# rflamino/monte_carlo_retirement

Hardware: AMD Instinct MI355X
Metric: paths/sec (whole node), config.json scenario, 833-month paths, success-count only (higher is better)
Workload: dtype f64

## Files before the change

monte_carlo_retirement_amd/csrc/build.py:

```python

from __future__ import annotations

import os
import shutil
import subprocess
import sys

HERE = os.path.dirname(os.path.abspath(__file__))
SOURCES = ["mcr_hip.hip", "mcr_aggregate.hip"]
HEADERS = ["mcr_device.h", "mcr_math.h", "mcr_tables.h", "mcr_numpy_rng.h", "mcr_numpy_tables.h", "mcr_screen.h", "mcr_host.h", os.path.join("..", "..", "include", "mcr.h")]
TARGET = os.path.join(HERE, "libmcr_hip.so")
ARCH = "gfx950"
FLAGS = ["-O3", "-std=c++17", "-fPIC", "-shared", "-ffp-contract=off", f"--offload-arch={ARCH}",
         "-Wall", "-Wno-unused-function"]


def hipcc() -> str:
    for cand in (os.environ.get("HIPCC"), shutil.which("hipcc"), "/opt/rocm/bin/hipcc"):
        if cand and os.path.exists(cand):
            return cand
    raise RuntimeError("hipcc not found (need ROCm)")


def is_stale() -> bool:
    if not os.path.exists(TARGET):
        return True
    t = os.path.getmtime(TARGET)
    deps = [os.path.join(HERE, s) for s in SOURCES + HEADERS] + [os.path.abspath(__file__)]
    return any(os.path.getmtime(d) > t for d in deps)


PER_SOURCE_FLAGS = {"mcr_hip.hip": ["-Xarch_device", "-fno-honor-nans"]}


def build(force: bool = False, verbose: bool = False, extra_flags=(), variant: str = "") -> str:
    if variant:
        return _build_to(os.path.join(HERE, f"libmcr_hip_{variant}.so"), f"_{variant}", verbose, extra_flags)
    if not force and not is_stale():
        return TARGET
    return _build_to(TARGET, "", verbose, extra_flags)


def _build_to(target: str, obj_suffix: str, verbose: bool, extra_flags) -> str:
    compile_flags = [f for f in FLAGS if f != "-shared"]
    objs = []
    for src in SOURCES:
        obj = os.path.join(HERE, src.replace(".hip", f"{obj_suffix}.o"))
        cmd = [hipcc(), *compile_flags, *PER_SOURCE_FLAGS.get(src, []), *extra_flags, "-c", "-o", obj, os.path.join(HERE, src)]
        if verbose:
            print(" ".join(cmd), flush=True)
        subprocess.check_call(cmd)
        objs.append(obj)
    cmd = [hipcc(), "-shared", "-fPIC", f"--offload-arch={ARCH}", "-o", target, *objs]
    if verbose:
        print(" ".join(cmd), flush=True)
    subprocess.check_call(cmd)
    return target


if __name__ == "__main__":
    build(force="--force" in sys.argv, verbose=True,
          extra_flags=["-Rpass-analysis=kernel-resource-usage"] if "--verbose" in sys.argv else [])
    print(TARGET)
```

monte_carlo_retirement_amd/csrc/mcr_device.h:

```cpp
#pragma once

#include <hip/hip_runtime.h>
#include <stdint.h>

#include "../../include/mcr.h"
#include "mcr_math.h"

#define MCR_MASKED_MOVE do { if (MM) asm volatile(""); } while (0)
namespace mcr {

constexpr double kEps = MCR_SMALL_EPSILON;
constexpr int kMPY = MCR_MONTHS_PER_YEAR;
constexpr int kBlock = 256;

struct DevStream {
    double amount;
    double keep;
    double amount_keep;
    int32_t start_month;
    int32_t end_month;
    int32_t indexed;
    int32_t lock_slot;
};
typedef const __attribute__((address_space(4))) DevStream* DevStreamTable;
// ... 532 lines not shown
        if (dust_s) { MCR_MASKED_MOVE; nbs = 0.0; ncs = 0.0; }
        if (dust_b) { MCR_MASKED_MOVE; nbb = 0.0; ncb = 0.0; }
        if (act) {
            MCR_MASKED_MOVE;
            if (sell1) { MCR_MASKED_MOVE; b1 = nbs; c1 = ncs; b2 = nbb; c2 = ncb; }
            else { MCR_MASKED_MOVE; b1 = nbb; c1 = ncb; b2 = nbs; c2 = ncs; }
        }
    }
}

template <bool TAXED, bool MM = true>
__device__ __forceinline__ void rebalance_path(const LaneParams& P, double& b1, double& c1, double& b2, double& c2) {
    const double total = b1 + b2;
    const double drift1 = b1 - total * P.alloc1;
    if ((total > kEps) && (fabs(drift1) > kEps)) {
        MCR_MASKED_MOVE;
        const bool sell1 = drift1 > 0.0;
        const double drift2 = b2 - total * P.alloc2;
        const double bs = sell1 ? b1 : b2, cs = sell1 ? c1 : c2;
        const double drift = sell1 ? drift1 : drift2;
        const double alloc_s = sell1 ? P.alloc1 : P.alloc2;
        const double rate_s = sell1 ? P.real_rate1 : P.real_rate2;
        const double inv_bs = recip_nr<false>(bs);
        double gross_sale;
        if (TAXED) {
            const double gain_fraction = div_by(fmax(0.0, bs - cs), bs, inv_bs);
            const double tax_per_dollar = gain_fraction * rate_s;
            const double denom = fmax(kEps, 1.0 - alloc_s * tax_per_dollar);
            gross_sale = fmin(bs, fdiv<false>(drift, denom));
        } else {
            gross_sale = fmin(bs, drift);
        }
        const double fraction_sold = div_by(gross_sale, bs, inv_bs);
        const double basis_removed = cs * fraction_sold;
        double net_purchase = gross_sale;
        if (TAXED) {
            const double taxable_gain = fmax(0.0, gross_sale - basis_removed);
            net_purchase = gross_sale - taxable_gain * rate_s;
        }
        const double nbs = bs - gross_sale;
        const double ncs = cs - basis_removed;
        double r1b = b1 + net_purchase, r1c = c1 + net_purchase;
        double r2b = b2 + net_purchase, r2c = c2 + net_purchase;
        if (sell1) { MCR_MASKED_MOVE; r1b = nbs; r1c = ncs; }
        else { MCR_MASKED_MOVE; r2b = nbs; r2c = ncs; }
        if (r1b <= kEps) { MCR_MASKED_MOVE; r1b = 0.0; r1c = 0.0; }
        if (r2b <= kEps) { MCR_MASKED_MOVE; r2b = 0.0; r2c = 0.0; }
        b1 = r1b; c1 = r1c; b2 = r2b; c2 = r2c;
    }
}

enum { kMonthEqualRates = 1 };

enum { kStreamsInRegs = 1 };


__device__ __forceinline__ bool wave_any(bool c) { return __builtin_amdgcn_ballot_w64(c) != 0ull; }

template <bool T1, bool T2 = T1, bool MM = true, bool UNIFORM = false>
__device__ __forceinline__ double capacity_tol(double b1, double c1, double r1, double b2, double c2, double r2) {
    double v1 = b1, v2 = b2;
    if (T1) v1 = __builtin_fma(-fmax(0.0, b1 - c1), r1, b1);
    if (T2) v2 = __builtin_fma(-fmax(0.0, b2 - c2), r2, b2);
    if (!UNIFORM) {
        if (b1 <= kEps) { MCR_MASKED_MOVE; v1 = 0.0; }
        if (b2 <= kEps) { MCR_MASKED_MOVE; v2 = 0.0; }
    }
    return v1 + v2;
}
template <bool MM = true, bool UNIFORM = false>
__device__ __forceinline__ void sell_fraction_tol(double phi, double& b1, double& c1, double& b2, double& c2) {
    double nb1 = __builtin_fma(-b1, phi, b1), nc1 = __builtin_fma(-c1, phi, c1);
    double nb2 = __builtin_fma(-b2, phi, b2), nc2 = __builtin_fma(-c2, phi, c2);
    if (!UNIFORM || wave_any(fmin(nb1, nb2) <= kEps)) {
        if (nb1 <= kEps) { MCR_MASKED_MOVE; nb1 = 0.0; nc1 = 0.0; }
        if (nb2 <= kEps) { MCR_MASKED_MOVE; nb2 = 0.0; nc2 = 0.0; }
    }
    if (!UNIFORM) {
        if (b1 <= kEps) { MCR_MASKED_MOVE; nb1 = b1; nc1 = c1; }
        if (b2 <= kEps) { MCR_MASKED_MOVE; nb2 = b2; nc2 = c2; }
    }
    b1 = nb1; c1 = nc1; b2 = nb2; c2 = nc2;
}
template <bool TAXED, bool MM = true, bool UNIFORM = false, bool EQR = false>
__device__ __forceinline__ void rebalance_tol(const DevParams& P, const LaneParams& L, double& b1, double& c1, double& b2, double& c2) {
    const double total = b1 + b2;
    const double drift1 = __builtin_fma(-total, P.alloc1, b1);
    if (UNIFORM && wave_any(fmin(total, fabs(drift1)) <= kEps)) {
        rebalance_tol<TAXED, MM, false, EQR>(P, L, b1, c1, b2, c2);
        return;
    }
    if (UNIFORM || ((total > kEps) && (fabs(drift1) > kEps))) {
        MCR_MASKED_MOVE;
        const bool sell1 = drift1 > 0.0;
        const double bs = sell1 ? b1 : b2, cs = sell1 ? c1 : c2;
        const double drift = fabs(drift1);
        double fraction_sold, net_purchase;
        if (TAXED) {
            const double rate_s = EQR ? L.real_rate1 : sell1 ? L.real_rate1 : L.real_rate2;
            const double ar_s = sell1 ? L.alloc1 : L.alloc2;
            const double G = fmax(0.0, bs - cs);
            fraction_sold = fmin(1.0, drift * recip_nr<false>(__builtin_fma(-ar_s, G, bs)));
            net_purchase = fraction_sold * __builtin_fma(-G, rate_s, bs);
        } else {
            fraction_sold = fmin(1.0, drift * recip_nr<false>(bs));
            net_purchase = fraction_sold * bs;
        }
        const double nbs = __builtin_fma(-bs, fraction_sold, bs);
        const double ncs = __builtin_fma(-cs, fraction_sold, cs);
        double r1b = b1 + net_purchase, r1c = c1 + net_purchase;
        double r2b = b2 + net_purchase, r2c = c2 + net_purchase;
        if (sell1) { MCR_MASKED_MOVE; r1b = nbs; r1c = ncs; }
        else { MCR_MASKED_MOVE; r2b = nbs; r2c = ncs; }
        if (!UNIFORM || wave_any(fmin(r1b, r2b) <= kEps)) {
            if (r1b <= kEps) { MCR_MASKED_MOVE; r1b = 0.0; r1c = 0.0; }
            if (r2b <= kEps) { MCR_MASKED_MOVE; r2b = 0.0; r2c = 0.0; }
        }
        b1 = r1b; c1 = r1c; b2 = r2b; c2 = r2c;
    }
}

template <bool STRICT = true, bool TAXED = true, bool ANNUAL = true, bool T1 = TAXED, bool T2 = TAXED, bool MM = true, bool TOL = false, bool EQR = false>
__device__ __forceinline__ bool annual_gain_taxes(const DevParams& P, const LaneParams& L, double& b1, double& c1,
                                                  double& b2, double& c2, double gain1, double gain2) {
    bool tax_failed = false;
    if (ANNUAL && P.any_annual_tax) {
        const double due1 = fmax(0.0, gain1) * P.annual_rate1;
        const double due2 = fmax(0.0, gain2) * P.annual_rate2;
        const double total_due = due1 + due2;
        const double cap1 = net_liquidation_value<STRICT, T1, MM>(b1, c1, L.real_rate1);
        const double cap2 = net_liquidation_value<STRICT, T2, MM>(b2, c2, L.real_rate2);
        const double cap = cap1 + cap2;
        const double pay = fmin(total_due, cap);
        tax_failed = pay < total_due - kEps;
        if (cap > kEps && pay > 0.0) {
            const double share1 = fdiv<STRICT>(cap1, cap);
            const double share2 = 1.0 - share1;
            double g, net1, net2;
            withdraw<STRICT, T1, MM>(b1, c1, pay * share1, L.real_rate1, g, net1);
            withdraw<STRICT, T2, MM>(b2, c2, pay * share2, L.real_rate2, g, net2);
            tax_failed = tax_failed || (net1 + net2 < total_due - kEps);
        }
    }
    if (STRICT) rebalance<true, TAXED, MM>(L, b1, c1, b2, c2);
    else if (TOL) rebalance_tol<TAXED, MM, false, EQR>(P, L, b1, c1, b2, c2);
    else rebalance_path<TAXED, MM>(L, b1, c1, b2, c2);
    return tax_failed;
}

template <bool ANNUAL = true, bool TOL = false>
__device__ __forceinline__ void market_step(double g1, double ginf, double g2, double& b1, double& b2,
                                            double& gacc1, double& gacc2, double& infl) {
    if (ANNUAL) {
        if (TOL) {
            gacc1 = __builtin_fma(b1, g1 - 1.0, gacc1);
            gacc2 = __builtin_fma(b2, g2 - 1.0, gacc2);
        } else {
            gacc1 += b1 * (g1 - 1.0);
            gacc2 += b2 * (g2 - 1.0);
        }
    }
    b1 *= g1;
    b2 *= g2;
    infl *= ginf;
}

}
```

monte_carlo_retirement_amd/csrc/mcr_hip.hip:

```cpp

#include <hip/hip_runtime.h>

#include <climits>
#include <cmath>
#include <cstdarg>
#include <cstdio>
#include <cstdlib>
#include <cstring>
#include <algorithm>
#include <mutex>
#include <thread>
#include <type_traits>
#include <utility>
#include <vector>

#include "mcr_device.h"
#include "mcr_numpy_rng.h"
#include "mcr_screen.h"
#include "mcr_host.h"

namespace mcr {

constexpr int kMaxSegments = 8;
constexpr int kRngHistorySchemes = 3;
struct KernelIO {
    uint64_t seed;
    uint64_t path_begin;
    uint64_t n_paths;
    const double* injected;
    mcr_outputs out;
    uint32_t stream_id;
    union { uint32_t n_entropy; uint32_t history_months; };
    union { uint32_t entropy[MCR_MAX_ENTROPY_WORDS]; struct { uint32_t history_block, history_scheme; }; };
    uint64_t child_offset;
    union {
        const uint32_t* path_seeds;
        const double* history;
    };
    double* snap;
    int64_t snap_stride;
    int32_t n_snap;
    int32_t snap_months[MCR_MAX_PROBE_CANDIDATES];
    int32_t cand_out[MCR_MAX_PROBE_CANDIDATES];
    int32_t seg_n_split, seg_n_full, seg_q;
    int32_t seg_blocks_per_cand;
    double* seg_state;
    int32_t seg_year[kMaxSegments + 1];
    int32_t seg_bid_base;
    unsigned int* seg_flags;
    int32_t seg_max_polls;
    int32_t fan_n;
    struct YearBins {
        const double* edges;
        const double* wr_edges;
        unsigned long long* trajectory;
        unsigned long long* real_trajectory;
        unsigned long long* wr;
        unsigned long long* final_success;
        int32_t n_bins, n_wr_bins;
    };
    struct FanRows {
        int64_t fan_stream_word;
        double* final_balance;
        double* years_to_ruin;
        int64_t row_stride;
    };
    struct RuleIO {
        double upper, lower, keep, grow, floor, ceiling;
        unsigned long long* year_counts;
        double* multipliers;
        int64_t stride;
    };
    struct FanRuleRows {
        FanRows rows;
        unsigned long long* year_counts;
    };
    union {
        double fan_expenses[MCR_MAX_EXPENSE_FANOUT];
        YearBins yb;
        int32_t fan_stream;
        FanRows fan_rows;
        struct { const uint32_t* path_list; const uint32_t* path_list_count; };
        RuleIO rule;
        FanRuleRows fan_rule;
    };
    uint64_t* fan_masks;
};
static_assert(sizeof(KernelIO::YearBins) <= sizeof(double) * MCR_MAX_EXPENSE_FANOUT, "the yearly-bins block must fit the bytes it overlays");
static_assert(sizeof(KernelIO::FanRows) <= sizeof(double) * MCR_MAX_EXPENSE_FANOUT, "the outcome rows must fit the bytes they overlay");
static_assert(sizeof(KernelIO::RuleIO) <= sizeof(double) * MCR_MAX_EXPENSE_FANOUT, "the spending rule must fit the bytes it overlays");
static_assert(sizeof(KernelIO::FanRuleRows) <= sizeof(double) * MCR_MAX_EXPENSE_FANOUT && offsetof(KernelIO::FanRuleRows, rows) == 0,
              "the rule fan-out's rows must fit the bytes they overlay, the outcome rows where every outcome probe reads them");
constexpr size_t kKernelIOArgOffset = (sizeof(DevParams) + alignof(KernelIO) - 1) / alignof(KernelIO) * alignof(KernelIO);
template <typename T> __device__ __forceinline__ T late_arg(size_t offset_in_io) {
    typedef const char __attribute__((address_space(4)))* KernArg;
    return *(const T __attribute__((address_space(4)))*)((KernArg)__builtin_amdgcn_kernarg_segment_ptr() + kKernelIOArgOffset + offset_in_io);
}
struct GridCell {
    DevParams p;
// ... 209 lines not shown
__device__ __forceinline__ void rule_year_binned(RuleState& r, const YearBinsRuleState& B, int year, bool valid, bool alive, double b1, double b2, double infl, uint64_t li) {
    rule_year_from(r, B.R, year, valid, alive, b1, b2, infl, li);
    if (B.L.mbins && valid && alive)
        atomicAdd(&B.L.buf[(B.k & 1) * B.L.row + 2 * B.L.cells + B.L.wcells + year_bins_cell(B.L.medges, B.L.mn, r.m)], 1u);
}
__device__ __forceinline__ void rule_bins_begin(YearBinsRuleState& B, const void* record) {
    const RuleBinsRecord* const rec = static_cast<const RuleBinsRecord*>(record);
    B.R.upper = rec->upper; B.R.lower = rec->lower; B.R.keep = rec->keep; B.R.grow = rec->grow; B.R.floor = rec->floor; B.R.ceiling = rec->ceiling;
    B.R.year_counts = rec->year_counts;
}
__device__ __forceinline__ void rule_bins_begin(YearBinsState&, const void*) {}
template <typename IO>
__device__ __forceinline__ void rule_year(NoRuleState&, const IO&, int, bool, bool, double, double, double, uint64_t) {}
template <typename IO>
__device__ __forceinline__ void rule_pad(const RuleState&, const IO& io, int year, bool valid, uint64_t li) {
    if (io.rule.multipliers && valid) store_bits(&io.rule.multipliers[(int64_t)year * io.rule.stride + (int64_t)li], kNanBits);
}
template <typename IO>
__device__ __forceinline__ void rule_pad(const NoRuleState&, const IO&, int, bool, uint64_t) {}
__device__ __forceinline__ void income_put(DevStream& S, const IncomeRegs& R) {
    S.amount = R.amount; S.amount_keep = R.amount_keep; S.start_month = R.start_month; S.end_month = R.end_month;
}

template <int MODE, int RNG, int TAXED, bool ANNUAL, bool INJ = false, int PHASE = 0, bool SPLIT = false, bool XS = false, bool EXACT = kExactMonthDefault, int GF = 0, int MF = 0, int SF = 0, bool OUT = false, bool LIST = false, int NPROD = 1, bool RULE = false>
__global__ __launch_bounds__((PHASE == 5 || PHASE == 6 || PHASE == 7 || PHASE == 8 || PHASE == 9 || PHASE == 10 || PHASE == 11) ? 64 * (MCR_MAX_EXPENSE_FANOUT + 1) : NPROD == 2 ? 3 * 64 : SPLIT ? 2 * kBlock : kBlock, SPLIT ? 4 : (MODE == 0 && RNG == 0 && (PHASE == 0 || PHASE == 3 || PHASE == 4)) ? 6 : ((MODE == 1 || MODE == 2) && RNG == 0 && !INJ) ? 5 : 4) void path_kernel(const DevParams P_arg, const KernelIO io,
                                                         const DevParams* __restrict__ cand_params) {
    static_assert(MODE != 3 || (PHASE == 0 && !SPLIT && !INJ), "the yearly-bins form is a whole-path launch on the engine's own streams");
    static_assert(!SPLIT || (MODE == 0 && RNG == 0 && !INJ), "the producer / consumer split exists for the count-only Philox variants");
    static_assert(!XS || (PHASE == 0 && !SPLIT && TAXED == 3 && ANNUAL), "extended stream lists run the generic whole-path form");
    static_assert(PHASE != 5 || SPLIT, "the expense fan-out is a producer / consumer form");
    static_assert(PHASE != 6 || SPLIT, "the grid fan-out is a producer / consumer form");
    static_assert(PHASE != 7 || SPLIT, "the contribution fan-out is a producer / consumer form");
    static_assert(PHASE != 8 || SPLIT, "the scenario fan-out is a producer / consumer form");
    static_assert(PHASE != 9 || SPLIT, "the assumption fan-out is a producer / consumer form");
    static_assert(PHASE != 10 || SPLIT, "the income fan-out is a producer / consumer form");
    static_assert(PHASE != 11 || (SPLIT && RULE), "the rule fan-out is a producer / consumer form of the rule kernels");
    static_assert(!OUT || PHASE == 8 || PHASE == 9 || PHASE == 10 || PHASE == 11, "outcome rows exist for the scenario, assumption, income and rule fan-outs");
    static_assert(!LIST || (MODE == 0 && RNG == (int)MCR_RNG_PHILOX && !ANNUAL && !INJ && PHASE == 0 && !XS), "path lists exist for the whole-path count-only Philox launches, split or not");
    static_assert(NPROD == 1 || (NPROD == 2 && SPLIT && LIST), "two producers exist for the split re-run of a screened launch");
    static_assert(!RULE || (RNG == (int)MCR_RNG_PHILOX && TAXED == 3 && !INJ && !XS && EXACT == kExactMonthDefault && GF == 0 && MF == 0 && SF == 0 && !LIST && NPROD == 1 &&
                            (((MODE == 0 || MODE == 1 || MODE == 3) && PHASE == 0 && !SPLIT && !OUT) || (MODE == 0 && PHASE == 11 && SPLIT) || (MODE == 0 && PHASE == 6 && SPLIT && !OUT))),
                  "the spending rule exists for the plain whole-path Philox launches, count-only, summary and yearly bins, and for the rule and the rule grid fan-outs, on the generic tax mask");
    constexpr bool kExpFan = PHASE == 5 || PHASE == 6;
    constexpr bool kConFan = PHASE == 7;
    constexpr bool kAsmFan = PHASE == 9;
    constexpr bool kStreamRegs = SPLIT && !kAsmFan && !(LIST && (SF & kStreamsInRegs) != 0);
    constexpr bool kIncFan = PHASE == 10;
    constexpr bool kRuleFan = PHASE == 11;
    constexpr bool kScnFan = PHASE == 8 || kAsmFan || kIncFan || kRuleFan;
    constexpr bool kFan = kExpFan || kConFan || kScnFan;
    constexpr bool kGrid = PHASE == 6;
    constexpr bool kRuleGrid = kGrid && RULE;
    constexpr bool kWaveRule = kRuleFan || kRuleGrid;
    constexpr bool kCand = PHASE == 2 || PHASE == 4 || kExpFan;
    constexpr bool kSliced = PHASE == 3 || PHASE == 4;
    constexpr bool kSIR = (SF & kStreamsInRegs) != 0;
    constexpr bool kScalarCounters = MODE == 0 && RNG == 0 && !ANNUAL && !INJ && (PHASE == 0 || PHASE == 3) && !SPLIT && !XS &&
                                     (kSIR || !(GF == (kGrowthNarrowExp | kGrowthRhoZero) && MF == 0));
    [[maybe_unused]] std::conditional_t<kScalarCounters, MonthCounters, NoMonthCounters> SC;
    [[maybe_unused]] std::conditional_t<kSIR, StreamRegs, NoStreamRegs> SR;
    [[maybe_unused]] std::conditional_t<kIncFan, IncomeRegs, NoIncomeRegs> IR;
    [[maybe_unused]] std::conditional_t<OUT, RuinMonth, NoRuinMonth> RM;
    [[maybe_unused]] std::conditional_t<RULE, RuleState, NoRuleState> RS;
    [[maybe_unused]] std::conditional_t<kWaveRule, FanRule, NoFanRule> FR;
    static_assert(!kSliced || (RNG == 0 && !INJ && !SPLIT && !XS), "time-sliced blocks exist for the plain Philox variants");
    static_assert(PHASE != 4 || MODE == 0, "the search probes count only");
    static_assert(TAXED >= 0 && TAXED <= 3, "TAXED is a two-bit mask");
    constexpr bool T1 = (TAXED & 1) != 0, T2 = (TAXED & 2) != 0, TANY = TAXED != 0;
    static_assert(!EXACT || XS || kExactMonthDefault, "the exact month is instantiated for the generic variants only");
    static_assert(GF == 0 || GF == kGrowthNarrowExp || GF == (kGrowthNarrowExp | kGrowthRhoZero), "growth forms: masks 0, 1 and 3");
    static_assert(GF == 0 || (MODE == 0 && RNG == (int)MCR_RNG_PHILOX && !ANNUAL && !INJ && (PHASE == 0 || PHASE == 3) && !SPLIT && !XS),
                  "growth forms exist for the per-path Philox count-only launches (kPerPathPhilox), whole path or time-sliced");
    static_assert(MF == 0 || MF == kMonthEqualRates, "month forms: masks 0 and 1");
    static_assert(MF == 0 || (MODE == 0 && RNG == (int)MCR_RNG_PHILOX && !ANNUAL && !INJ && (PHASE == 0 || PHASE == 3) && (!SPLIT || LIST) && !XS && !EXACT),
                  "month forms exist for the kernels that have growth forms and for the split re-run of a screened launch, in the tolerance form of the month");
    static_assert(!(MF & kMonthEqualRates) || TAXED == 3, "equal realized-gains rates: both assets are taxed");
    constexpr bool EQR = (MF & kMonthEqualRates) != 0;
    static_assert(SF == 0 || SF == kStreamsInRegs, "stream forms: masks 0 and 1");
    static_assert(SF == 0 || (MODE == 0 && RNG == (int)MCR_RNG_PHILOX && !ANNUAL && !INJ && (PHASE == 0 || PHASE == 3) && (!SPLIT || LIST) && !XS && !EXACT),
                  "stream forms exist for the kernels that have growth forms and for the split re-run of a screened launch, in the tolerance form of the month");
    constexpr bool TOL = !EXACT;
    constexpr bool MM = !SPLIT || kFan || NPROD == 2 || LIST;
    constexpr bool kFastMonth = TOL && MM && kUniformFixups;
    constexpr int kPaths = (kFan || NPROD == 2) ? 64 : kBlock;
    const int kThreads = kFan ? (int)blockDim.x : NPROD == 2 ? 3 * 64 : SPLIT ? 2 * kBlock : kBlock;
    const int tid = SPLIT ? (int)(threadIdx.x & (kPaths - 1)) : (int)threadIdx.x;
    const int fan_j = kFan ? __builtin_amdgcn_readfirstlane((int)(threadIdx.x >> 6)) : 0;
    const bool producer = kFan ? fan_j == io.fan_n : (SPLIT && threadIdx.x >= (unsigned)kPaths);
    int seg = -1, seg_block = 0;
    unsigned int path_block = blockIdx.x, cand = (PHASE == 2 || kGrid) ? blockIdx.y : 0u;
    if (kSliced) {
        const int S = io.seg_n_split, F = io.seg_n_full, bid = (int)blockIdx.x + io.seg_bid_base;
        unsigned int lb = (unsigned)bid;
        if (bid < S) { seg = 0; seg_block = bid; }
        else if (bid >= S + F) { const int k = bid - S - F; seg = 1 + k / S; seg_block = k % S; lb = (unsigned)seg_block; }
        if (PHASE == 4) { cand = lb / (unsigned)io.seg_blocks_per_cand; path_block = lb % (unsigned)io.seg_blocks_per_cand; }
        else path_block = lb;
    }
    if constexpr (LIST) {
        if ((uint64_t)blockIdx.x * kPaths >= (uint64_t)*io.path_list_count) return;
    }
    const GridCell* cell = kRuleGrid ? &(reinterpret_cast<const RuleGridCell*>(cand_params) + cand)->cell
                           : kGrid ? reinterpret_cast<const GridCell*>(cand_params) + cand : nullptr;
    const DevParams& P = kGrid ? cell->p : (kCand && !kFan) ? cand_params[cand] : P_arg;
    const int snap_c = kGrid ? cell->snap : (int)cand;
    constexpr bool kStaged = RNG == (int)MCR_RNG_PHILOX && !INJ;
    constexpr bool kHistory = (RNG == (int)MCR_RNG_HISTORY || RNG == kRngHistorySchemes) && !INJ;
    __shared__ __align__(16) double tab_s[kHistory ? 1 : kTabDoubles];
    constexpr int kStageLen = (kAsmFan ? kPartsPerPair : 6) * kPaths;
    constexpr int kStageRing = SPLIT ? 2 : 1;
    __shared__ __align__(16) double stage_s[kStaged ? kStageRing * kStageLen : 1];
    constexpr bool kBins = MODE == 3;
    constexpr bool kSumLds = (MODE == 1 || MODE == 2) && kStaged;
    __shared__ __align__(16) double sum_s[kSumLds ? 3 * kBlock : 1];
    extern __shared__ __align__(16) unsigned char smem_raw[];
#ifdef MCR_K1_TIMELINE
    const unsigned long long tl_t0 = wall_clock64();
#endif
    double* tab = kHistory ? reinterpret_cast<double*>(smem_raw) : tab_s;
    load_math_tables<(GF & kGrowthNarrowExp) != 0>(tab, threadIdx.x, kThreads);
    ZigTables zig{nullptr, nullptr, nullptr, nullptr};
    if (RNG == (int)MCR_RNG_NUMPY) { zig = load_zig_tables(smem_raw, threadIdx.x, kThreads); zig.math_tab = tab; }
    [[maybe_unused]] const double* const hist_tab = reinterpret_cast<const double*>(smem_raw);
    [[maybe_unused]] std::conditional_t<kHistory, HistoryCursor, NoHistoryCursor> HC;
    if constexpr (kHistory) {
        constexpr int kRowsPerThread = MCR_MAX_HISTORY_MONTHS / kBlock;
        static_assert(kRowsPerThread * kBlock == MCR_MAX_HISTORY_MONTHS, "every row of the longest record has a thread");
        HC = history_cursor();
        __syncthreads();
        const int H = (int)io.history_months;
        double g[kRowsPerThread][3];
#pragma unroll
        for (int i = 0; i < kRowsPerThread; ++i) {
            const int k = (int)threadIdx.x + i * kBlock;
            g[i][0] = g[i][1] = g[i][2] = 0.0;
            if (k < H) {
                const double ze = io.history[3 * k + 0], zi = io.history[3 * k + 1], zp = io.history[3 * k + 2];
                g[i][0] = monthly_gross(P.a1, P.b1, ze, tab);
                g[i][1] = monthly_gross(P.ainf, P.binf, zi, tab);
                g[i][2] = g[i][1] * monthly_gross(P.aprem, P.bprem, zp, tab);
            }
        }
        __syncthreads();
        double* const G = reinterpret_cast<double*>(smem_raw);
#pragma unroll
        for (int i = 0; i < kRowsPerThread; ++i) {
            const int k = (int)threadIdx.x + i * kBlock;
            if (k < H) { G[3 * k + 0] = g[i][0]; G[3 * k + 1] = g[i][1]; G[3 * k + 2] = g[i][2]; }
        }
    }
    double* stage = stage_s + (kStaged ? tid : 0);
    double* sum_col = sum_s + (kSumLds ? tid : 0);
    double* lock_lds = reinterpret_cast<double*>(smem_raw + (RNG == (int)MCR_RNG_NUMPY ? (size_t)kZigLdsBytes
                                                             : kHistory ? (size_t)io.history_months * 3u * sizeof(double) : (size_t)0));
    unsigned int* blk = reinterpret_cast<unsigned int*>(lock_lds + (size_t)P.n_lock_slots * kPaths * (kFan ? io.fan_n : 1));
    if (kFan && !producer) lock_lds += (size_t)fan_j * P.n_lock_slots * kPaths;
    const int ry = P.retirement_years;
    const int n_blk = kFan ? MCR_MAX_EXPENSE_FANOUT : 1 + (ry + 2) + (ry + 1);
    const int n_hist = ((PHASE == 0 || PHASE == 3) && io.out.hist_bins != nullptr) ? io.out.hist_n_bins : 0;
    for (int k = threadIdx.x; k < n_blk + n_hist; k += kThreads) blk[k] = 0u;
    constexpr bool kBinsRule = kBins && RULE;
    [[maybe_unused]] std::conditional_t<kBins, std::conditional_t<kBinsRule, YearBinsRuleState, YearBinsState>, NoYearBins> YB;
    if constexpr (kBins) {
        year_bins_plan(YB.L, io.yb, cand_params, blk + n_blk + n_hist);
        rule_bins_begin(YB, cand_params);
        YB.k = 0; YB.last = 0.0;
// ... 200 lines not shown
        c1 = b1; c2 = b2;
        contrib = rec->monthly_contribution;
        scn_expenses = rec->monthly_expenses;
    } else if constexpr (kRuleFan) {
        const RuleRecord* const rec = reinterpret_cast<const RuleRecord*>(cand_params) + fan_j;
        const double rec_balance = rec->initial_balance;
        b1 = rec_balance * P.alloc1;
        b2 = rec_balance - b1;
        c1 = b1; c2 = b2;
        contrib = rec->monthly_contribution;
        scn_expenses = rec->monthly_expenses;
        FR.upper = rec->upper; FR.lower = rec->lower; FR.keep = rec->keep; FR.grow = rec->grow; FR.floor = rec->floor; FR.ceiling = rec->ceiling;
        unsigned long long* const yc = late_arg<unsigned long long*>(offsetof(KernelIO, fan_rule) + offsetof(KernelIO::FanRuleRows, year_counts));
        FR.year_counts = yc ? yc + (size_t)fan_j * (size_t)P.retirement_years * MCR_RULE_N_COUNTS : nullptr;
    } else if constexpr (kRuleGrid) {
        const RuleGridCell* const rec = reinterpret_cast<const RuleGridCell*>(cand_params) + cand;
        FR.upper = rec->upper; FR.lower = rec->lower; FR.keep = rec->keep; FR.grow = rec->grow; FR.floor = rec->floor; FR.ceiling = rec->ceiling;
        unsigned long long* const yc = rec->year_counts;
        FR.year_counts = yc ? yc + (size_t)fan_j * (size_t)P.retirement_years * MCR_RULE_N_COUNTS : nullptr;
    } else if constexpr (kScnFan) {
        const mcr_scenario* const scn = reinterpret_cast<const mcr_scenario*>(cand_params) + fan_j;
        const double scn_balance = scn->initial_balance;
        b1 = scn_balance * P.alloc1;
        b2 = scn_balance - b1;
        c1 = b1; c2 = b2;
        contrib = scn->monthly_contribution;
        scn_expenses = scn->monthly_expenses;
    }
    if (PHASE == 1) while (snap_i < io.n_snap && io.snap_months[snap_i] == 0) save_snapshot();
    constexpr int kSegFixedFields = MODE >= 1 ? 14 : 9;
    double seg_start_balance = 0.0, seg_infl_ret = 0.0;
    auto seg_at = [&](int f) { return io.seg_state + ((size_t)seg_block * (size_t)(kSegFixedFields + P.n_lock_slots) + (size_t)f) * kBlock + (size_t)tid; };
    __shared__ int seg_ok_s;
    bool seg_resumed = false;
    int y_begin = 0, y_end = ry;
    unsigned long long seg_state_flags = 0ull;
    if (kSliced && seg >= 0) {
        y_end = io.seg_year[seg + 1];
        if (seg > 0) {
            if (threadIdx.x == 0) {
                const unsigned int* f = io.seg_flags + (size_t)seg_block * (size_t)io.seg_q + (size_t)(seg - 1);
                unsigned int v = 0u;
                for (int spin = 0; spin < io.seg_max_polls; ++spin) {
                    if ((v = __hip_atomic_load(f, __ATOMIC_ACQUIRE, __HIP_MEMORY_SCOPE_AGENT)) != 0u) break;
                    __builtin_amdgcn_s_sleep(32);
                }
                seg_ok_s = v == 1u;
            }
            __syncthreads();
            seg_resumed = seg_ok_s != 0;
            if (seg_resumed) {
                __builtin_amdgcn_fence(__ATOMIC_ACQUIRE, "agent");
                b1 = *seg_at(0); b2 = *seg_at(1); c1 = *seg_at(2); c2 = *seg_at(3);
                if (ANNUAL) { gacc1 = *seg_at(4); gacc2 = *seg_at(5); }
                infl = *seg_at(6);
                seg_state_flags = f64_bits(*seg_at(7));
                const unsigned long long cw = f64_bits(*seg_at(8));
                carry.w2 = (uint32_t)cw; carry.w3 = (uint32_t)(cw >> 32);
                for (int k = 0; k < P.n_lock_slots; ++k) lock_lds[(size_t)k * kBlock + tid] = *seg_at(kSegFixedFields + k);
                if (MODE >= 1) {
                    seg_start_balance = *seg_at(9); seg_infl_ret = *seg_at(10);
                    sum_col[0] = *seg_at(11); sum_col[kBlock] = *seg_at(12); sum_col[2 * kBlock] = *seg_at(13);
                }
                y_begin = io.seg_year[seg];
                const int r0 = wm + kMPY * y_begin;
                if (r0 >= prio_t3) __builtin_amdgcn_s_setprio(0);
                else if (r0 >= prio_t2) __builtin_amdgcn_s_setprio(1);
                else if (r0 >= prio_t1) __builtin_amdgcn_s_setprio(2);
                if constexpr (kScalarCounters) { SC.prio_next = prio_from(prio_t1, prio_t2, prio_t3, r0 - (r0 & 1)); SC.row = r0; }
                if (r0 & 1) begin_month(r0 - 1);
            }
        }
    }

    if (kCand && !seg_resumed) {
        const int c = snap_c;
        b1 = *snap_at(c, 0); b2 = *snap_at(c, 1); c1 = *snap_at(c, 2); c2 = *snap_at(c, 3);
        gacc1 = *snap_at(c, 4); gacc2 = *snap_at(c, 5); infl = *snap_at(c, 6); contrib = *snap_at(c, 7);
        pre_fail = *snap_at(c, 8) != 0.0;
        const unsigned long long cw = f64_bits(*snap_at(c, 9));
        carry.w2 = (uint32_t)cw; carry.w3 = (uint32_t)(cw >> 32);
        if (wm & 1) begin_month(wm - 1);
    }
    for (int m = 1; m <= ((kCand || (kSliced && seg_resumed)) ? 0 : wm); ++m) {
        if constexpr (kScalarCounters) ++SC.moy;
        if (P.contrib_grows && year_opens(SC, m - 1) && m > 1) {
            asm volatile("");
            contrib *= P.contrib_growth_factor;
        }
        begin_month(m - 1);
        double g1, ginf, g2;
        growth(m - 1, g1, ginf, g2);
        market_step<ANNUAL, TOL>(g1, ginf, g2, b1, b2, gacc1, gacc2, infl);
        const double k1 = contrib * P.alloc1;
        const double k2 = contrib - k1;
        b1 += k1; c1 += k1; b2 += k2; c2 += k2;
        if (TOL) rebalance_tol<TANY, MM, kFastMonth, EQR>(P, L, b1, c1, b2, c2);
        else rebalance_path<TANY, MM>(L, b1, c1, b2, c2);
        if (year_closes(SC, m)) {
            if constexpr (kScalarCounters) SC.moy = 0;
            pre_fail |= annual_gain_taxes<false, TANY, ANNUAL, T1, T2, MM, TOL, EQR>(P, L, b1, c1, b2, c2, gacc1, gacc2);
            put_sample(t_idx++, b1 + b2, infl);
            gacc1 = 0.0; gacc2 = 0.0;
        }
        if (PHASE == 1 && snap_i < io.n_snap && m == io.snap_months[snap_i]) save_snapshot();
    }
    if (PHASE == 1) return;
    if constexpr (kScalarCounters) { if (!(kSliced && seg_resumed)) SC.row = wm; }
    double start_balance = b1 + b2;
    double infl_ret = infl;
    if (kSliced && seg_resumed) { start_balance = seg_start_balance; infl_ret = seg_infl_ret; t_idx = P.trajectory_len - ry + y_begin; }
    else if (wm > 0 && wm % kMPY != 0) put_sample(t_idx++, start_balance, infl_ret);
    rule_begin(RS, start_balance, infl_ret);

    double fy_gross = 0.0, fy_real = 0.0;
    bool alive = !pre_fail;
    bool succeeded = !pre_fail;
    unsigned long long ytr_bits = pre_fail ? f64_bits(0.0) : kNanBits;
    if (kSumLds && !(kSliced && seg_resumed)) { sum_col[0] = 0.0; sum_col[kBlock] = 0.0; store_bits(&sum_col[2 * kBlock], ytr_bits); }
    DevStream S0 = {}, S1 = {};
    if constexpr (kIncFan) {
        const IncomeRecord* const rec = reinterpret_cast<const IncomeRecord*>(cand_params) + fan_j;
        IR.k = io.fan_stream;
        IR.amount = rec->amount; IR.amount_keep = rec->amount_keep; IR.start_month = rec->start_month; IR.end_month = rec->end_month;
    }
    if (kStreamRegs) {
        if (P.n_streams > 0) S0 = P.streams[0];
        if (P.n_streams > 1) S1 = P.streams[1];
        if constexpr (kIncFan) {
            if (IR.k == 0) income_put(S0, IR);
            if (IR.k == 1) income_put(S1, IR);
        }
        if (TOL) {
            asm volatile("" : "+s"(S0.amount_keep), "+s"(S0.start_month), "+s"(S0.end_month), "+s"(S0.indexed), "+s"(S0.lock_slot));
            asm volatile("" : "+s"(S1.amount_keep), "+s"(S1.start_month), "+s"(S1.end_month), "+s"(S1.indexed), "+s"(S1.lock_slot));
        } else {
            asm volatile("" : "+s"(S0.amount), "+s"(S0.keep), "+s"(S0.start_month), "+s"(S0.end_month), "+s"(S0.indexed), "+s"(S0.lock_slot));
            asm volatile("" : "+s"(S1.amount), "+s"(S1.keep), "+s"(S1.start_month), "+s"(S1.end_month), "+s"(S1.indexed), "+s"(S1.lock_slot));
        }
    }
    if constexpr (kSIR) {
        auto to_row = [&](int32_t m) { return m > INT32_MAX - wm ? INT32_MAX : m + wm; };
        auto window_months = [](int first, int end) { return end > first ? (unsigned)(end - first) : 0u; };
        SR = StreamRegs{0.0, 0.0, 0, 0, 0u, 0u};
        if (P.n_streams > 0) { SR.a0 = P.streams[0].amount_keep; SR.s0 = to_row(P.streams[0].start_month); SR.n0 = window_months(SR.s0, to_row(P.streams[0].end_month)); }
        if (P.n_streams > 1) { SR.a1 = P.streams[1].amount_keep; SR.s1 = to_row(P.streams[1].start_month); SR.n1 = window_months(SR.s1, to_row(P.streams[1].end_month)); }
        asm volatile("" : "+s"(SR.a0), "+s"(SR.s0), "+s"(SR.n0));
        asm volatile("" : "+s"(SR.a1), "+s"(SR.s1), "+s"(SR.n1));
    }
    const double fan_expenses = kGrid ? cell->levels[fan_j] : kExpFan ? io.fan_expenses[fan_j] : 0.0;
    int ruin_bin = pre_fail ? 0 : -1;
    if constexpr (OUT) RM.month = pre_fail ? 0 : -1;
    int done_years = 0;
    int year = 0;
    if (kSliced && seg_resumed) {
        alive = (seg_state_flags & 1ull) != 0ull;
        succeeded = (seg_state_flags & 2ull) != 0ull;
        ruin_bin = (int)((seg_state_flags >> 8) & 0xFFFFull) - 1;
        done_years = (int)(seg_state_flags >> 24);
        year = y_begin;
    }
    for (; year < (kSliced ? y_end : ry); ++year) {
        if (!SPLIT && __builtin_amdgcn_ballot_w64(alive) == 0ull) break;
        if (SPLIT) { lane_alive = alive; if (wg_dead) break; }
        if constexpr (kWaveRule) rule_year_from(RS, FR, year, valid, alive, b1, b2, infl, li);
        else if constexpr (kBinsRule) rule_year_binned(RS, YB, year, valid, alive, b1, b2, infl, li);
        else
        rule_year(RS, io, year, valid, alive, b1, b2, infl, li);
        double tg1 = 0.0, tg2 = 0.0, treal = 0.0;
        bool yfail = false;
        int fail_rmi = 0;
        for (int mi = 0; mi < kMPY; ++mi) {
            const int rmi = year * kMPY + mi;
            begin_month(month_row(SC, wm + rmi));
            if (alive && !yfail) {
                double g1, ginf, g2;
                if (kStaged) growth(month_row(SC, wm + rmi), g1, ginf, g2);
                const double price = infl;
                const double expenses = (kExpFan ? rule_scaled(RS, fan_expenses) : kScnFan ? rule_scaled(RS, scn_expenses) : rule_scaled(RS, P.monthly_expenses)) * price;
                double income = TOL ? expenses : 0.0;
                auto stream_income = [&](const DevStream& S) {
                    if (rmi < S.start_month || rmi >= S.end_month) return;
                    double nominal = 0.0;
                    if (S.indexed) {
                        if (TOL) { income = __builtin_fma(-S.amount_keep, price, income); return; }
                        nominal = S.amount * price;
                    } else if (!XS || S.lock_slot < P.n_lock_slots) {
                        double* slot = lock_lds + (size_t)S.lock_slot * kPaths + tid;
                        if (rmi == S.start_month) *slot = (TOL ? S.amount_keep : S.amount) * price;
                        nominal = *slot;
                    } else {
                        double* slot = P.lock_overflow + (size_t)(S.lock_slot - P.n_lock_slots) * (size_t)P.lock_stride + (size_t)local;
                        if (rmi == S.start_month) *slot = (TOL ? S.amount_keep : S.amount) * price;
                        nominal = *slot;
                    }
                    if (TOL) income -= nominal;
                    else income += nominal * S.keep;
                };
                int s = 0;
                if (kStreamRegs) {
                    if (P.n_streams > 0) stream_income(S0);
                    if (P.n_streams > 1) stream_income(S1);
                    s = 2;
                }
                if constexpr (kSIR && SPLIT && LIST) {
                    if ((unsigned)(wm + rmi - SR.s0) < SR.n0) { asm volatile(""); income = __builtin_fma(-SR.a0, price, income); }
                    if ((unsigned)(wm + rmi - SR.s1) < SR.n1) { asm volatile(""); income = __builtin_fma(-SR.a1, price, income); }
                } else
                if constexpr (kSIR) {
                    if ((unsigned)(SC.row - SR.s0) < SR.n0) { asm volatile(""); income = __builtin_fma(-SR.a0, price, income); }
                    if ((unsigned)(SC.row - SR.s1) < SR.n1) { asm volatile(""); income = __builtin_fma(-SR.a1, price, income); }
                } else if constexpr (kIncFan) {
                    for (; s < P.n_streams; ++s) {
                        DevStream S = P.streams[s];
                        if (s == IR.k) income_put(S, IR);
                        stream_income(S);
                    }
                } else for (; s < P.n_streams; ++s) stream_income(P.streams[s]);
                if (XS && P.n_extra_streams > 0) {
                    const DevStreamTable xs = (DevStreamTable)P.extra_streams;
                    for (int x = 0; x < P.n_extra_streams; ++x) {
                        DevStream S;
                        S.amount = xs[x].amount; S.keep = xs[x].keep; S.amount_keep = xs[x].amount_keep; S.start_month = xs[x].start_month;
                        S.end_month = xs[x].end_month; S.indexed = xs[x].indexed; S.lock_slot = xs[x].lock_slot;
                        stream_income(S);
                    }
                }
                const double need = fmax(0.0, TOL ? income : expenses - income);
                bool stop = false;
                if (b1 + b2 <= kEps && need > kEps) {
                    yfail = true; stop = true;
                }
                auto tol_month = [&](auto fast_tag) {
                    constexpr bool FAST = decltype(fast_tag)::value;
                    const double cap = capacity_tol<T1, T2, MM, FAST>(b1, c1, L.real_rate1, b2, c2, L.real_rate2);
                    const double target = fmin(need, cap);
                    bool fail = need > kEps && target < need - kEps;
                    double phi = target * recip_nr<false>(cap);
                    double gross = phi * (FAST ? b1 + b2 : (b1 > kEps ? b1 : 0.0) + (b2 > kEps ? b2 : 0.0));
                    if (!FAST && wave_any(!(cap > kEps))) {
                        if (!(cap > kEps)) {
                            MCR_MASKED_MOVE;
                            double cap1, cap2, gw1, nw1, gw2, nw2;
                            net_liquidation_values2<T1, T2, MM>(b1, c1, L.real_rate1, b2, c2, L.real_rate2, cap1, cap2);
                            const double xcap = cap1 + cap2, xtarget = fmin(need, xcap);
// ... 3673 lines not shown
```

Measured before the change: 441.5 million.

## Add paired-month consumer loop with event scheduling and mask-based seller select

For the split producer/consumer stream-form launch, the consumer now processes months in pairs, loading six staged growth factors per handover and synchronising once per pair instead of once per month. Stream windows and priority switches are driven by a precomputed event cursor held in scalar registers, not tested every month. Rebalancing can pick seller values with a ballot mask and raw v_cndmask inline asm. This cuts barrier and per-month control overhead, at the cost of a large duplicated code path, a specialised static_assert scope, and hand-written asm that is fragile.

```diff
diff --git a/monte_carlo_retirement_amd/csrc/build.py b/monte_carlo_retirement_amd/csrc/build.py
--- a/monte_carlo_retirement_amd/csrc/build.py
+++ b/monte_carlo_retirement_amd/csrc/build.py
@@ -8,7 +8,7 @@
 
 HERE = os.path.dirname(os.path.abspath(__file__))
 SOURCES = ["mcr_hip.hip", "mcr_aggregate.hip"]
-HEADERS = ["mcr_device.h", "mcr_math.h", "mcr_tables.h", "mcr_numpy_rng.h", "mcr_numpy_tables.h", "mcr_screen.h", "mcr_host.h", os.path.join("..", "..", "include", "mcr.h")]
+HEADERS = ["mcr_device.h", "mcr_events.h", "mcr_math.h", "mcr_tables.h", "mcr_numpy_rng.h", "mcr_numpy_tables.h", "mcr_screen.h", "mcr_host.h", os.path.join("..", "..", "include", "mcr.h")]
 TARGET = os.path.join(HERE, "libmcr_hip.so")
 ARCH = "gfx950"
 FLAGS = ["-O3", "-std=c++17", "-fPIC", "-shared", "-ffp-contract=off", f"--offload-arch={ARCH}",
diff --git a/monte_carlo_retirement_amd/csrc/mcr_device.h b/monte_carlo_retirement_amd/csrc/mcr_device.h
--- a/monte_carlo_retirement_amd/csrc/mcr_device.h
+++ b/monte_carlo_retirement_amd/csrc/mcr_device.h
@@ -638,23 +638,40 @@
     }
     b1 = nb1; c1 = nc1; b2 = nb2; c2 = nc2;
 }
-template <bool TAXED, bool MM = true, bool UNIFORM = false, bool EQR = false>
+__device__ __forceinline__ void seller_select3(bool sell1, double a1, double a2, double b1, double b2, double c1, double c2, double& a, double& b, double& c) {
+    const unsigned long long m = __builtin_amdgcn_ballot_w64(sell1);
+    auto bits = [](double x) { return (unsigned long long)__double_as_longlong(x); };
+    const unsigned long long a1b = bits(a1), a2b = bits(a2), b1b = bits(b1), b2b = bits(b2), c1b = bits(c1), c2b = bits(c2);
+    uint32_t alo, ahi, blo, bhi, clo, chi;
+    asm("s_nop 1\n\tv_cndmask_b32_e64 %0, %7, %6, %18\n\tv_cndmask_b32_e64 %1, %9, %8, %18\n\tv_cndmask_b32_e64 %2, %11, %10, %18\n\t"
+        "v_cndmask_b32_e64 %3, %13, %12, %18\n\tv_cndmask_b32_e64 %4, %15, %14, %18\n\tv_cndmask_b32_e64 %5, %17, %16, %18"
+        : "=&v"(alo), "=&v"(ahi), "=&v"(blo), "=&v"(bhi), "=&v"(clo), "=&v"(chi)
+        : "v"((uint32_t)a1b), "v"((uint32_t)a2b), "v"((uint32_t)(a1b >> 32)), "v"((uint32_t)(a2b >> 32)),
+          "v"((uint32_t)b1b), "v"((uint32_t)b2b), "v"((uint32_t)(b1b >> 32)), "v"((uint32_t)(b2b >> 32)),
+          "v"((uint32_t)c1b), "v"((uint32_t)c2b), "v"((uint32_t)(c1b >> 32)), "v"((uint32_t)(c2b >> 32)), "s"(m));
+    auto f64 = [](uint32_t hi, uint32_t lo) { return __longlong_as_double((long long)(((unsigned long long)hi << 32) | lo)); };
+    a = f64(ahi, alo); b = f64(bhi, blo); c = f64(chi, clo);
+}
+template <bool TAXED, bool MM = true, bool UNIFORM = false, bool EQR = false, bool MASKSEL = false>
 __device__ __forceinline__ void rebalance_tol(const DevParams& P, const LaneParams& L, double& b1, double& c1, double& b2, double& c2) {
     const double total = b1 + b2;
     const double drift1 = __builtin_fma(-total, P.alloc1, b1);
     if (UNIFORM && wave_any(fmin(total, fabs(drift1)) <= kEps)) {
-        rebalance_tol<TAXED, MM, false, EQR>(P, L, b1, c1, b2, c2);
+        rebalance_tol<TAXED, MM, false, EQR, MASKSEL>(P, L, b1, c1, b2, c2);
         return;
     }
     if (UNIFORM || ((total > kEps) && (fabs(drift1) > kEps))) {
         MCR_MASKED_MOVE;
         const bool sell1 = drift1 > 0.0;
-        const double bs = sell1 ? b1 : b2, cs = sell1 ? c1 : c2;
+        constexpr bool kMaskSel = MASKSEL && TAXED && EQR;
+        [[maybe_unused]] double m_ar = 0.0, m_bs = 0.0, m_cs = 0.0;
+        if constexpr (kMaskSel) seller_select3(sell1, L.alloc1, L.alloc2, b1, b2, c1, c2, m_ar, m_bs, m_cs);
+        const double bs = kMaskSel ? m_bs : sell1 ? b1 : b2, cs = kMaskSel ? m_cs : sell1 ? c1 : c2;
         const double drift = fabs(drift1);
         double fraction_sold, net_purchase;
         if (TAXED) {
             const double rate_s = EQR ? L.real_rate1 : sell1 ? L.real_rate1 : L.real_rate2;
-            const double ar_s = sell1 ? L.alloc1 : L.alloc2;
+            const double ar_s = kMaskSel ? m_ar : sell1 ? L.alloc1 : L.alloc2;
             const double G = fmax(0.0, bs - cs);
             fraction_sold = fmin(1.0, drift * recip_nr<false>(__builtin_fma(-ar_s, G, bs)));
             net_purchase = fraction_sold * __builtin_fma(-G, rate_s, bs);
diff --git a/monte_carlo_retirement_amd/csrc/mcr_events.h b/monte_carlo_retirement_amd/csrc/mcr_events.h
--- /dev/null
+++ b/monte_carlo_retirement_amd/csrc/mcr_events.h
@@ -0,0 +1,45 @@
+#pragma once
+#include <cstdint>
+
+#if defined(__HIPCC__) || defined(__CUDACC__)
+#define MCR_EV_FN __host__ __device__ __forceinline__
+#else
+#define MCR_EV_FN inline
+#endif
+#if defined(__HIP_DEVICE_COMPILE__)
+#define MCR_EV_SCALAR(x) do { (x) = __builtin_amdgcn_readfirstlane(x); asm volatile("" : "+s"(x)); } while (0)
+#else
+#define MCR_EV_SCALAR(x) ((void)(x))
+#endif
+
+struct EventPlan { int t1, t2, t3; int s0; unsigned n0; int s1; unsigned n1; };
+struct EventRow { int next; int w0, w1; };
+
+MCR_EV_FN int event_close_row(int s, unsigned n) {
+    const unsigned c = (unsigned)s + n;
+    return (c < (unsigned)s || c >= (unsigned)INT32_MAX) ? INT32_MAX : (int)c;
+}
+MCR_EV_FN int event_next(const EventPlan& e, int from) {
+    int r = INT32_MAX;
+    auto take = [&](int x) { if (x >= from && x < r) r = x; };
+    take(e.t1); take(e.t2); take(e.t3);
+    if (e.n0 != 0u) { take(e.s0); take(event_close_row(e.s0, e.n0)); }
+    if (e.n1 != 0u) { take(e.s1); take(event_close_row(e.s1, e.n1)); }
+    return r;
+}
+MCR_EV_FN EventRow event_begin(const EventPlan& e) {
+    EventRow ev{event_next(e, 0), 0, 0};
+    MCR_EV_SCALAR(ev.w0); MCR_EV_SCALAR(ev.w1); MCR_EV_SCALAR(ev.next);
+    return ev;
+}
+MCR_EV_FN int event_fire(EventRow& ev, const EventPlan& e, int row) {
+    ev.w0 = (unsigned)(row - e.s0) < e.n0 ? 1 : 0;
+    ev.w1 = (unsigned)(row - e.s1) < e.n1 ? 1 : 0;
+    ev.next = event_next(e, row + 1);
+    MCR_EV_SCALAR(ev.w0); MCR_EV_SCALAR(ev.w1); MCR_EV_SCALAR(ev.next);
+    return row == e.t1 ? 2 : row == e.t2 ? 1 : row == e.t3 ? 0 : -1;
+}
+
+struct PairCursor { int pair; unsigned off; };
+MCR_EV_FN bool pair_votes(const PairCursor& c, int vote_pairs) { return (c.pair & (vote_pairs - 1)) == 0; }
+MCR_EV_FN void pair_advance(PairCursor& c, unsigned stage_len) { ++c.pair; c.off ^= stage_len; }
diff --git a/monte_carlo_retirement_amd/csrc/mcr_hip.hip b/monte_carlo_retirement_amd/csrc/mcr_hip.hip
--- a/monte_carlo_retirement_amd/csrc/mcr_hip.hip
+++ b/monte_carlo_retirement_amd/csrc/mcr_hip.hip
@@ -15,6 +15,7 @@
 #include <vector>
 
 #include "mcr_device.h"
+#include "mcr_events.h"
 #include "mcr_numpy_rng.h"
 #include "mcr_screen.h"
 #include "mcr_host.h"
@@ -390,6 +391,9 @@
     constexpr bool TOL = !EXACT;
     constexpr bool MM = !SPLIT || kFan || NPROD == 2 || LIST;
     constexpr bool kFastMonth = TOL && MM && kUniformFixups;
+    constexpr bool kPairs = SPLIT && LIST;
+    static_assert(!kPairs || (MODE == 0 && PHASE == 0 && kSIR && TOL && MM && !ANNUAL && !OUT && !RULE && !kFan),
+                  "the paired consumer is stated for the re-run's own forms: a whole-path count-only launch, the tolerance month, the stream form");
     constexpr int kPaths = (kFan || NPROD == 2) ? 64 : kBlock;
     const int kThreads = kFan ? (int)blockDim.x : NPROD == 2 ? 3 * 64 : SPLIT ? 2 * kBlock : kBlock;
     const int tid = SPLIT ? (int)(threadIdx.x & (kPaths - 1)) : (int)threadIdx.x;
@@ -756,7 +760,7 @@
         carry.w2 = (uint32_t)cw; carry.w3 = (uint32_t)(cw >> 32);
         if (wm & 1) begin_month(wm - 1);
     }
-    for (int m = 1; m <= ((kCand || (kSliced && seg_resumed)) ? 0 : wm); ++m) {
+    for (int m = 1; m <= ((kPairs || kCand || (kSliced && seg_resumed)) ? 0 : wm); ++m) {
         if constexpr (kScalarCounters) ++SC.moy;
         if (P.contrib_grows && year_opens(SC, m - 1) && m > 1) {
             asm volatile("");
@@ -834,7 +838,150 @@
         done_years = (int)(seg_state_flags >> 24);
         year = y_begin;
     }
-    for (; year < (kSliced ? y_end : ry); ++year) {
+    if constexpr (kPairs) {
+        static_assert(kMPY % 2 == 0, "a retirement year is a whole number of pairs");
+        constexpr bool kSel = true;
+        const EventPlan EP{prio_t1, prio_t2, prio_t3, SR.s0, SR.n0, SR.s1, SR.n1};
+        EventRow EV = event_begin(EP);
+        PairCursor PC{0, 0u};
+        int row = 0;
+        int dead = 0;
+        double f0 = 0.0, f1 = 0.0, f2 = 0.0, f3 = 0.0, f4 = 0.0, f5 = 0.0;
+        auto handover = [&]() __attribute__((always_inline)) {
+            if (dead) return;
+            if (pair_votes(PC, kSplitVotePairs)) {
+                const int any = __syncthreads_or(__builtin_amdgcn_ballot_w64(lane_alive) != 0ull ? 1 : 0);
+                if (__builtin_amdgcn_readfirstlane(any) == 0) { dead = 1; return; }
+            } else __syncthreads();
+            const double* const c = stage + PC.off;
+            f0 = c[0]; f1 = c[kPaths]; f2 = c[2 * kPaths]; f3 = c[3 * kPaths]; f4 = c[4 * kPaths]; f5 = c[5 * kPaths];
+            pair_advance(PC, (unsigned)kStageLen);
+        };
+        auto events = [&]() __attribute__((always_inline)) {
+            if (row == EV.next) {
+                const int p = event_fire(EV, EP, row);
+                if (p == 2) __builtin_amdgcn_s_setprio(2);
+                else if (p == 1) __builtin_amdgcn_s_setprio(1);
+                else if (p == 0) __builtin_amdgcn_s_setprio(0);
+            }
+        };
+        auto factors = [&](int half, double& g1, double& ginf, double& g2) __attribute__((always_inline)) {
+            g1 = half ? f3 : f0; ginf = half ? f4 : f1; g2 = half ? f5 : f2;
+        };
+        int moy = 0;
+        auto acc_month = [&](int m, int half) __attribute__((always_inline)) {
+            if (P.contrib_grows && moy == 0 && m > 1) {
+                asm volatile("");
+                contrib *= P.contrib_growth_factor;
+            }
+            events();
+            double g1, ginf, g2;
+            factors(half, g1, ginf, g2);
+            market_step<ANNUAL, TOL>(g1, ginf, g2, b1, b2, gacc1, gacc2, infl);
+            const double k1 = contrib * P.alloc1;
+            const double k2 = contrib - k1;
+            b1 += k1; c1 += k1; b2 += k2; c2 += k2;
+            rebalance_tol<TANY, MM, kFastMonth, EQR, kSel>(P, L, b1, c1, b2, c2);
+            if (++moy == kMPY) {
+                moy = 0;
+                pre_fail |= annual_gain_taxes<false, TANY, ANNUAL, T1, T2, MM, TOL, EQR>(P, L, b1, c1, b2, c2, gacc1, gacc2);
+                gacc1 = 0.0; gacc2 = 0.0;
+            }
+            ++row;
+        };
+        {
+            int m = 1;
+            for (; m < wm; m += 2) { handover(); acc_month(m, 0); acc_month(m + 1, 1); }
+            if (m == wm) { handover(); acc_month(m, 0); }
+        }
+        alive = !pre_fail; succeeded = !pre_fail; ruin_bin = pre_fail ? 0 : -1;
+        const int ye_mi = kMPY - 1 - wm % kMPY;
+        auto ret_month = [&](int mi, int half, bool& yfail) __attribute__((always_inline)) {
+            events();
+            if (alive && !yfail) {
+                const double price = infl;
+                const double expenses = P.monthly_expenses * price;
+                double income = expenses;
+                if (EV.w0) { asm volatile(""); income = __builtin_fma(-SR.a0, price, income); }
+                if (EV.w1) { asm volatile(""); income = __builtin_fma(-SR.a1, price, income); }
+                const double need = fmax(0.0, income);
+                bool stop = false;
+                if (b1 + b2 <= kEps && need > kEps) {
+                    yfail = true; stop = true;
+                }
+                auto tol_month = [&](auto fast_tag) __attribute__((always_inline)) {
+                    constexpr bool FAST = decltype(fast_tag)::value;
+                    const double cap = capacity_tol<T1, T2, MM, FAST>(b1, c1, L.real_rate1, b2, c2, L.real_rate2);
+                    const double target = fmin(need, cap);
+                    bool fail = need > kEps && target < need - kEps;
+                    double phi = target * recip_nr<false>(cap);
+                    if (!FAST && wave_any(!(cap > kEps))) {
+                        if (!(cap > kEps)) {
+                            MCR_MASKED_MOVE;
+                            double cap1, cap2, gw1, nw1, gw2, nw2;
+                            net_liquidation_values2<T1, T2, MM>(b1, c1, L.real_rate1, b2, c2, L.real_rate2, cap1, cap2);
+                            const double xcap = cap1 + cap2, xtarget = fmin(need, xcap);
+                            const double prop1 = xcap > kEps ? fdiv<false>(cap1, xcap) : P.alloc1;
+                            withdraw2<T1, T2, MM>(b1, c1, xtarget * prop1, L.real_rate1, gw1, nw1,
+                                                  b2, c2, xtarget * (1.0 - prop1), L.real_rate2, gw2, nw2);
+                            fail = need > kEps && (xtarget < need - kEps || nw1 + nw2 < need - kEps);
+                            phi = 0.0;
+                        }
+                    }
+                    if (fail) yfail = true;
+                    sell_fraction_tol<MM, FAST>(phi, b1, c1, b2, c2);
+                    rebalance_tol<TANY, MM, kFastMonth, EQR, kSel>(P, L, b1, c1, b2, c2);
+                    if (!yfail && mi == ye_mi) {
+                        const bool tf = annual_gain_taxes<false, TANY, ANNUAL, T1, T2, MM, true, EQR>(P, L, b1, c1, b2, c2, gacc1, gacc2);
+                        gacc1 = 0.0; gacc2 = 0.0;
+                        yfail = yfail || tf;
+                    }
+                };
+                if (!stop) {
+                    double g1, ginf, g2;
+                    factors(half, g1, ginf, g2);
+                    market_step<ANNUAL, TOL>(g1, ginf, g2, b1, b2, gacc1, gacc2, infl);
+                    if (kFastMonth && !wave_any(fmin(b1, b2) <= P.fast_floor)) {
+                        tol_month(std::true_type{});
+                    } else {
+                        if (b1 + b2 <= kEps && need > kEps) {
+                            MCR_MASKED_MOVE;
+                            b1 = fmax(0.0, b1); b2 = fmax(0.0, b2);
+                            yfail = true; stop = true;
+                        }
+                        if (!stop) tol_month(std::false_type{});
+                    }
+                }
+            }
+            ++row;
+        };
+        auto ret_years = [&](auto odd_tag) __attribute__((always_inline)) {
+            constexpr bool ODD = decltype(odd_tag)::value;
+            for (; year < ry; ++year) {
+                lane_alive = alive;
+                if (dead) break;
+                bool yfail = false;
+#pragma nounroll
+                for (int mi = 0; mi < kMPY; mi += 2) {
+                    if constexpr (ODD) {
+                        ret_month(mi, 1, yfail);
+                        handover();
+                        ret_month(mi + 1, 0, yfail);
+                    } else {
+                        handover();
+                        ret_month(mi, 0, yfail);
+                        ret_month(mi + 1, 1, yfail);
+                    }
+                }
+                if (alive) {
+                    if (yfail) { succeeded = false; ruin_bin = 1 + year; alive = false; }
+                    else done_years = year + 1;
+                }
+            }
+        };
+        if (wm & 1) ret_years(std::true_type{}); else ret_years(std::false_type{});
+    }
+    for (; !kPairs && year < (kSliced ? y_end : ry); ++year) {
         if (!SPLIT && __builtin_amdgcn_ballot_w64(alive) == 0ull) break;
         if (SPLIT) { lane_alive = alive; if (wg_dead) break; }
         if constexpr (kWaveRule) rule_year_from(RS, FR, year, valid, alive, b1, b2, infl, li);
```

After: 453.3 million, median of 6. +2.7%, better.
